# BaratiLab/MeshDQN

Hardware: AMD Instinct MI355X
Metric: env steps/sec (ys930 ~2k-tri) (higher is better)
Workload: dtype f64; 1 GPU; ys930 (876 vertices / 1570 triangles), 128 envs per GPU, S3 env step (remesh+smooth+interp+forces+state+1 IPCS step+Q-fwd); mesh=ys930, envs_per_gpu=128, parallelism=dp1 (independent envs sharded, no data-path collective)

## Files before the change

meshdqn_amd/csrc/mdq_ipcs_entry.hip:

```cpp
namespace mdq {

#ifdef MDQ_AT_TRACE
extern "C" MDQ_API int mdq_at_trace_host(long long* out, int reset) {
  if (hipMemcpyFromSymbol(out, HIP_SYMBOL(mdq_at_trace_buf), sizeof(long long) * 16) != hipSuccess) return -1;
  if (reset) { long long z[16] = {0}; if (hipMemcpyToSymbol(HIP_SYMBOL(mdq_at_trace_buf), z, sizeof z) != hipSuccess) return -1; }
  return 0;
}
extern "C" MDQ_API int mdq_pt_trace_host(long long* out, int reset) {
  if (hipMemcpyFromSymbol(out, HIP_SYMBOL(mdq_pt_trace_buf), sizeof(long long) * 16) != hipSuccess) return -1;
  if (reset) { long long z[16] = {0}; if (hipMemcpyToSymbol(HIP_SYMBOL(mdq_pt_trace_buf), z, sizeof z) != hipSuccess) return -1; }
  return 0;
}
extern "C" MDQ_API int mdq_ct_trace_host(long long* out, int reset) {
  if (hipMemcpyFromSymbol(out, HIP_SYMBOL(mdq_ct_trace_buf), sizeof(long long) * 16) != hipSuccess) return -1;
  if (reset) { long long z[16] = {0}; if (hipMemcpyToSymbol(HIP_SYMBOL(mdq_ct_trace_buf), z, sizeof z) != hipSuccess) return -1; }
  return 0;
}
#endif

static thread_local std::string g_err;

static int fail(const char* what, hipError_t e) {
  g_err = std::string(what) + ": " + hipGetErrorString(e);
  return -1;
// ... 66 lines not shown
  if (int rc = ensure_tables()) return rc;
  const size_t stage_bytes = 52 * (size_t)d->NT + 9 * (size_t)d->N2 + 9 * (size_t)d->NV + 64;
  hipError_t e;
  const size_t list_bytes = 2 * ((size_t)d->N2 + 1 + 6 * (size_t)d->NT + (size_t)d->NV + 1 + 3 * (size_t)d->NT) + 2;
  if (stage_bytes + list_bytes <= 156 * 1024 && 6 * (size_t)d->NT <= 65535) {
    const size_t bytes = stage_bytes + list_bytes;
    e = hipFuncSetAttribute(reinterpret_cast<const void*>(&setup_matfree_kernel<true, true>),
                            hipFuncAttributeMaxDynamicSharedMemorySize, (int)bytes);
    if (e != hipSuccess) return fail("setup_matfree_kernel attribute", e);
    hipLaunchKernelGGL((setup_matfree_kernel<true, true>), dim3(d->B), dim3(SWG), bytes, (hipStream_t)stream, *d);
  } else if (stage_bytes <= 156 * 1024) {
    e = hipFuncSetAttribute(reinterpret_cast<const void*>(&setup_matfree_kernel<true>), hipFuncAttributeMaxDynamicSharedMemorySize,
                            (int)stage_bytes);
    if (e != hipSuccess) return fail("setup_matfree_kernel attribute", e);
    hipLaunchKernelGGL(setup_matfree_kernel<true>, dim3(d->B), dim3(SWG), stage_bytes, (hipStream_t)stream, *d);
  } else if (const size_t idx_bytes = 12 * (size_t)d->NT + (size_t)d->N2 + 9 * (size_t)d->NV + 64;
             idx_bytes <= 156 * 1024 && d->N2 <= 65535 && std::getenv("MDQ_SETUP_UNSTAGED") == nullptr) {
    e = hipFuncSetAttribute(reinterpret_cast<const void*>(&setup_matfree_kernel<true, false, false>),
                            hipFuncAttributeMaxDynamicSharedMemorySize, (int)idx_bytes);
    if (e != hipSuccess) return fail("setup_matfree_kernel attribute", e);
    hipLaunchKernelGGL((setup_matfree_kernel<true, false, false>), dim3(d->B), dim3(SWG), idx_bytes, (hipStream_t)stream, *d);
  } else {
    hipLaunchKernelGGL(setup_matfree_kernel<false>, dim3(d->B), dim3(SWG), 0, (hipStream_t)stream, *d);
  }
  e = hipGetLastError();
  if (e != hipSuccess) return fail("setup_matfree_kernel launch", e);
  return 0;
}

static int ipcs_evolve_impl(const mdq_ipcs_desc* d, int32_t nsteps, double* drag, double* lift, int32_t* iters,
                            const double* inflow_scale, void* stream, double* kernel_ms, int fresh = 0,
                            const mdq_inflow_profile* prof = nullptr);

static int evolve_profile_checked(const char* entry, int fresh, const mdq_ipcs_desc* d, int32_t nsteps, double* drag, double* lift,
                                  int32_t* iters, const mdq_inflow_profile* prof, void* stream) {
  if (prof) {
    const auto bad = [entry](const char* what) { return fail_msg(std::string(entry) + what); };
    if (prof->NIN <= 0 || prof->NIR <= 0) return bad(": NIN and NIR must be positive");
    if (!prof->n_inlet || !prof->inlet_dofs || !prof->n_rows || !prof->rows || !prof->values)
      return bad(": incomplete inflow profile (n_inlet, inlet_dofs, n_rows, rows, values)");
    if (d && (!d->cell_dofs || !d->g2_ptr || !d->g2_src || !d->bcu_flag || !d->bcu_gx || !d->geom || !d->lift1 || !d->lift3))
      return bad(": incomplete descriptor (cell_dofs, g2_ptr, g2_src, bcu_flag, bcu_gx, geom, lift1, lift3)");
  }
  return ipcs_evolve_impl(d, nsteps, drag, lift, iters, nullptr, stream, nullptr, fresh, prof);
}

int mdq_ipcs_evolve_profile(const mdq_ipcs_desc* d, int32_t nsteps, double* drag, double* lift, int32_t* iters,
                            const mdq_inflow_profile* prof, void* stream) {
  return evolve_profile_checked("mdq_ipcs_evolve_profile", 0, d, nsteps, drag, lift, iters, prof, stream);
}

int mdq_ipcs_evolve_fresh_profile(const mdq_ipcs_desc* d, int32_t nsteps, double* drag, double* lift, int32_t* iters,
                                  const mdq_inflow_profile* prof, void* stream) {
  return evolve_profile_checked("mdq_ipcs_evolve_fresh_profile", 1, d, nsteps, drag, lift, iters, prof, stream);
}

int mdq_ipcs_build_inlet_map(const mdq_ipcs_desc* d, int32_t NIN, int32_t NIR, const int32_t* n_ref, const double* inlet_y,
                             int32_t* n_inlet, int32_t* inlet_dofs, int32_t* n_rows, int32_t* rows, int32_t* map_status,
                             void* stream) {
  if (!d || d->B <= 0 || d->NV <= 0 || d->NT <= 0 || d->NE <= 0 || d->N2 != d->NV + d->NE)
    return fail_msg("mdq_ipcs_build_inlet_map: bad batch sizes");
  if (!d->nv || !d->nt || !d->ne || !d->coords || !d->cell_dofs || !d->cell_outflow || !d->bcu_flag || !d->bcu_gx)
    return fail_msg("mdq_ipcs_build_inlet_map: incomplete descriptor (nv, nt, ne, coords, cell_dofs, cell_outflow, bcu_flag, bcu_gx)");
  if (d->N2 > MAP_BITS)
    return fail_msg("mdq_ipcs_build_inlet_map: N2 > " + std::to_string(MAP_BITS) + " (the inlet map serves the meshes of operator mode 3)");
  if (NIN <= 0 || NIN > MAP_NIN || NIR <= 0)
    return fail_msg("mdq_ipcs_build_inlet_map: NIN must be in 1 .. " + std::to_string(MAP_NIN) + " and NIR positive");
  if (!n_ref || !inlet_y || !n_inlet || !inlet_dofs || !n_rows || !rows || !map_status)
    return fail_msg("mdq_ipcs_build_inlet_map: null table (n_ref, inlet_y, n_inlet, inlet_dofs, n_rows, rows, map_status)");
  hipLaunchKernelGGL(inlet_map_kernel, dim3(d->B), dim3(MWG), 0, (hipStream_t)stream, *d, NIN, NIR, n_ref, inlet_y, n_inlet,
                     inlet_dofs, n_rows, rows, map_status);
  hipError_t e = hipGetLastError();
  if (e != hipSuccess) return fail("inlet_map_kernel launch", e);
  return 0;
}

int mdq_ipcs_evolve(const mdq_ipcs_desc* d, int32_t nsteps, double* drag, double* lift, int32_t* iters,
                    void* stream) {
  return ipcs_evolve_impl(d, nsteps, drag, lift, iters, nullptr, stream, nullptr);
}

int mdq_ipcs_evolve_inflow(const mdq_ipcs_desc* d, int32_t nsteps, double* drag, double* lift, int32_t* iters,
                           const double* inflow_scale, void* stream) {
  return ipcs_evolve_impl(d, nsteps, drag, lift, iters, inflow_scale, stream, nullptr);
}

int mdq_ipcs_evolve_fresh(const mdq_ipcs_desc* d, int32_t nsteps, double* drag, double* lift, int32_t* iters,
                          const double* inflow_scale, void* stream) {
  return ipcs_evolve_impl(d, nsteps, drag, lift, iters, inflow_scale, stream, nullptr, 1);
}

int mdq_ipcs_evolve_timed(const mdq_ipcs_desc* d, int32_t nsteps, double* drag, double* lift, int32_t* iters,
                          void* stream, double* kernel_ms) {
  if (!kernel_ms) return fail_msg("kernel_ms is required");
  if (d && d->mode != 3 && d->mode != -1) return fail_msg("per-kernel timing exists for the three-kernel mode 3 only");
  return ipcs_evolve_impl(d, nsteps, drag, lift, iters, nullptr, stream, kernel_ms);
}

static int ipcs_evolve_impl(const mdq_ipcs_desc* d, int32_t nsteps, double* drag, double* lift, int32_t* iters,
                            const double* inflow_scale, void* stream, double* kernel_ms, int fresh,
                            const mdq_inflow_profile* prof) {
  if (int rc = check_desc(d)) return rc;
  if (nsteps <= 0) return fail_msg("nsteps must be positive");
  if (!drag || !lift) return fail_msg("drag/lift output pointers are required");
  if (int rc = ensure_tables()) return rc;
  const LdsPlan P = lds_plan(d->N2, d->NV, d->NSE1);
  const size_t LDS_MAX = 160 * 1024, red_bytes = 64 * sizeof(double);
  const bool pg = red_bytes + P.prs_vec_bytes > LDS_MAX;
  const bool k1_lds = !pg && !d->pd_enabled && red_bytes + P.prs_vec_bytes + P.prs_mat_bytes <= LDS_MAX;
  int mode = d->mode;
  const size_t tile_bytes = tile_lds_bytes(*d);
  if (mode == 6) return fail_msg("unknown operator mode 6");
  if (mode < 0 || mode > 7) {
    mode = 0;
    if (red_bytes + P.vel1_bytes <= LDS_MAX) mode = 1;
    if (red_bytes + P.vel2_bytes <= LDS_MAX && d->N2 <= MF_ROWS * WG) mode = 2;
    if (d->mode != -2 && red_bytes + P.vel3_bytes <= LDS_MAX && d->N2 <= MF_ROWS * WG) mode = 3;
    if (mode == 0 && d->cell_outflow && ((d->mf_scat && d->mf_tptr) || (d->g2_ptr && d->g2_src)) && std::getenv("MDQ_NO_MODE5") == nullptr) mode = 5;
    if (mode == 0) {
      const int ncu = team_cus((hipStream_t)stream);
      if (!pg && 2 * TEAM * d->B <= ncu) mode = 4;
    }
    if (mode == 5 && !pg && std::getenv("MDQ_NO_TEAM_TILES") == nullptr) {
      if (TEAM * d->B <= team_cus((hipStream_t)stream)) mode = 7;
    }
  }
  if (kernel_ms && mode != 3) return fail_msg("per-kernel timing exists for the three-kernel mode 3 only");
  if (prof && mode != 2 && mode != 3)
    return fail_msg("mdq_ipcs_evolve_profile: operator mode " + std::to_string(mode) + " runs the steps of a call inside one kernel; "
                    "an inflow profile is served by the per-step path (operator modes 2 and 3, or mdq_ipcs_setup_matfree + "
                    "mdq_ipcs_evolve one step at a time)");
  if (fresh && mode != 3) {
    hipLaunchKernelGGL(reset_history_kernel, dim3((d->B + 63) / 64), dim3(64), 0, (hipStream_t)stream, *d, iters);
    if (hipError_t e_ = hipGetLastError(); e_ != hipSuccess) return fail("reset_history_kernel launch", e_);
  }
  if (mode == 3 && (red_bytes + P.vel3_bytes > LDS_MAX || d->N2 > MF_ROWS * WG))
    return fail_msg("mode 3 needs N2 <= 3584 and three velocity vectors in LDS");
  if (mode == 2 && (red_bytes + P.vel2_bytes > LDS_MAX || d->N2 > MF_ROWS * WG))
    return fail_msg("matrix-free tile mode needs N2 <= 3584 and the x stage + element tile in LDS");
  if (mode == 1 && red_bytes + P.vel1_bytes > LDS_MAX) return fail_msg("LDS gather vectors do not fit");
  if ((mode == 5 || mode == 7) && (!d->cell_outflow || !((d->mf_scat && d->mf_tptr) || (d->g2_ptr && d->g2_src))))
    return fail_msg("modes 5 / 7 need cell_outflow and the tile maps (mf_scat, mf_tptr) or the dof <- slot lists (g2_ptr, g2_src)");
  if (pg && mode != 0 && mode != 5)
    return fail_msg("mesh too large for the LDS-resident pressure vectors of this operator mode (use mode -1, 0 or 5)");
  size_t u = pg ? tl_extra_bytes(d->NV) + sizeof(double) * NAG * NAG : P.prs_vec_bytes + (k1_lds ? P.prs_mat_bytes : 0);
  const size_t vel = mode == 3 ? P.vel3_bytes : (mode == 2 ? P.vel2_bytes : (mode == 1 ? P.vel1_bytes : ((mode == 5 || mode == 7) ? tile_bytes : 0)));
  if (vel > u) u = vel;
  const size_t lds = red_bytes + u;
  hipError_t e;
  hipStream_t st = (hipStream_t)stream;
  if (mode == 3) {
    const size_t lds_v = red_bytes + P.vel3_bytes;
    const size_t lds_p = red_bytes + P.prs_vec_bytes + (k1_lds ? P.prs_mat_bytes : 0);
    const size_t lds_c = red_bytes + 2 * sizeof(double2) * (size_t)P.N2p + sizeof(double) * (size_t)P.NVp;
    static const hipError_t attr_err = [] {
      hipError_t e_ = hipFuncSetAttribute(reinterpret_cast<const void*>(&at_velocity_kernel<WG, MF_ROWS, AT_PAIR>),
                                          hipFuncAttributeMaxDynamicSharedMemorySize, 160 * 1024);
      if (e_ == hipSuccess)
        e_ = hipFuncSetAttribute(reinterpret_cast<const void*>(&at_velocity_kernel<768, 5, 1>),
                                 hipFuncAttributeMaxDynamicSharedMemorySize, 160 * 1024);
      if (e_ == hipSuccess)
        e_ = hipFuncSetAttribute(reinterpret_cast<const void*>(&at_pressure_kernel<true>),
                                 hipFuncAttributeMaxDynamicSharedMemorySize, 160 * 1024);
      if (e_ == hipSuccess)
        e_ = hipFuncSetAttribute(reinterpret_cast<const void*>(&at_pressure_kernel<false>),
                                 hipFuncAttributeMaxDynamicSharedMemorySize, 160 * 1024);
      if (e_ == hipSuccess)
        e_ = hipFuncSetAttribute(reinterpret_cast<const void*>(&at_pressure_kernel<false, 1024>),
                                 hipFuncAttributeMaxDynamicSharedMemorySize, 160 * 1024);
      if (e_ == hipSuccess)
        e_ = hipFuncSetAttribute(reinterpret_cast<const void*>(&at_correction_kernel),
                                 hipFuncAttributeMaxDynamicSharedMemorySize, 160 * 1024);
      return e_;
    }();
    if (attr_err != hipSuccess) return fail("hipFuncSetAttribute(mode 3 kernels)", attr_err);
    static const int vel_wg = [] {
      const char* s_ = std::getenv("MDQ_AT_WG");
      const int w_ = s_ ? std::atoi(s_) : 768;
      return w_ == 512 ? 512 : 768;
    }();
    hipEvent_t ev[4] = {nullptr, nullptr, nullptr, nullptr};
    if (kernel_ms) {
      for (int i = 0; i < 4; ++i)
        if ((e = hipEventCreate(&ev[i])) != hipSuccess) return fail("hipEventCreate", e);
      kernel_ms[0] = kernel_ms[1] = kernel_ms[2] = 0.0;
    }
    for (int step = 0; step < nsteps; ++step) {
      if (prof)
        if ((e = launch_inflow_lift(d, prof, nsteps, step, st)) != hipSuccess) return fail("inflow_lift_kernel launch", e);
      if (kernel_ms) hipEventRecord(ev[0], st);
      if (vel_wg == 768)
        hipLaunchKernelGGL((at_velocity_kernel<768, 5, 1>), dim3(d->B), dim3(768), lds_v, st, *d, iters, inflow_scale, nsteps, step, fresh);
      else
        hipLaunchKernelGGL((at_velocity_kernel<WG, MF_ROWS, AT_PAIR>), dim3(d->B), dim3(WG), lds_v, st, *d, iters, inflow_scale, nsteps, step, fresh);
      if (kernel_ms) hipEventRecord(ev[1], st);
      if (d->pd_enabled)
        hipLaunchKernelGGL((at_pressure_kernel<false, 1024>), dim3(d->B), dim3(1024), lds_p, st, *d, iters, fresh && step == 0);
      else if (k1_lds)
        hipLaunchKernelGGL(at_pressure_kernel<true>, dim3(d->B), dim3(WG), lds_p, st, *d, iters, fresh && step == 0);
      else
        hipLaunchKernelGGL(at_pressure_kernel<false>, dim3(d->B), dim3(WG), lds_p, st, *d, iters, fresh && step == 0);
      if (kernel_ms) hipEventRecord(ev[2], st);
      hipLaunchKernelGGL(at_correction_kernel, dim3(d->B), dim3(WG), lds_c, st, *d, nsteps, step, drag, lift, iters, inflow_scale, fresh);
      if (kernel_ms) {
        hipEventRecord(ev[3], st);
        if ((e = hipEventSynchronize(ev[3])) != hipSuccess) return fail("hipEventSynchronize", e);
        for (int i = 0; i < 3; ++i) {
          float ms = 0.f;
          hipEventElapsedTime(&ms, ev[i], ev[i + 1]);
          kernel_ms[i] += ms;
        }
      }
    }
    if (kernel_ms)
      for (int i = 0; i < 4; ++i) hipEventDestroy(ev[i]);
    e = hipGetLastError();
  } else {
    const EvolveArgs a{d, lds, nsteps, drag, lift, iters, inflow_scale, st, prof};
    if (mode == 2)
      e = part_launch_mf(k1_lds, a);
    else if (mode == 4 || mode == 5 || mode == 7)
      e = part_launch_tiles(mode, k1_lds, pg, a);
    else
      e = part_launch_assembled(mode, k1_lds, pg, a);
  }
  if (e != hipSuccess) return fail("evolve_kernel launch", e);
  return 0;
}

int mdq_probe_forces(const mdq_ipcs_desc* d, int32_t nfields, const double* u, const double* p, double* drag,
                     double* lift, void* stream) {
  if (!d || d->B <= 0 || d->N2 != d->NV + d->NE || !d->coords || !d->cell_dofs || !d->af_facets)
    return fail_msg("mdq_probe_forces: incomplete mesh descriptor");
  if (nfields <= 0 || !u || !p || !drag || !lift) return fail_msg("bad probe arguments");
  if (int rc = ensure_tables()) return rc;
  hipLaunchKernelGGL(probe_kernel, dim3(d->B), dim3(WG), 0, (hipStream_t)stream, *d, nfields, u, p, drag, lift);
  hipError_t e = hipGetLastError();
  if (e != hipSuccess) return fail("probe_kernel launch", e);
  return 0;
}

}
```

meshdqn_amd/csrc/mdq_ipcs_mode3.hip:

```cpp
#ifndef MDQ_CORR_MX0_INTERLEAVE
#define MDQ_CORR_MX0_INTERLEAVE false
#endif
#ifndef MDQ_PCG_REGM
#define MDQ_PCG_REGM 1
#endif
namespace mdq {

__device__ __forceinline__ double f2d(float f) {
  asm volatile("" : "+v"(f));
  return (double)f;
}


constexpr int AT_PAIR = 2;

template <int TPAIR = AT_PAIR>
struct AtMetaT {
  int w[TPAIR][6];
  Geo g[TPAIR];
};
using AtMeta = AtMetaT<AT_PAIR>;

template <int TW = WG, int TPAIR = AT_PAIR>
__device__ __forceinline__ void at_prefetch(const EnvView& v, AtMetaT<TPAIR>& m, int round) {
#pragma unroll
  for (int j = 0; j < TPAIR; ++j) {
    const int e = threadIdx.x + (round * TPAIR + j) * TW;
    if (e < v.nt) {
#pragma unroll
      for (int i = 0; i < 6; ++i) m.w[j][i] = v.mf_scat[i * v.NT + e];
      m.g[j] = load_geo(v, e);
    }
  }
}

template <bool INTERLEAVE, int TW = WG, int TPAIR = AT_PAIR, class ElemOp>
__device__ __forceinline__ void atomic_accumulate(const EnvView& v, double* Yd, AtMetaT<TPAIR>& m, ElemOp op) {
  const int nrounds = (v.nt + TPAIR * TW - 1) / (TPAIR * TW);
  for (int round = 0; round < nrounds; ++round) {
    if (INTERLEAVE) {
      double2 ye[TPAIR][6];
      int dof[TPAIR][6];
#pragma unroll
      for (int j = 0; j < TPAIR; ++j) {
        const int e = threadIdx.x + (round * TPAIR + j) * TW;
        if (e < v.nt) {
          ElemIdx E;
#pragma unroll
          for (int i = 0; i < 6; ++i) E.dof[i] = dof[j][i] = m.w[j][i] & 0xFFF;
          op(e, m.g[j], E, ((m.w[j][0] >> 28) & 3) - 1, ye[j]);
        }
      }
#pragma unroll
      for (int j = 0; j < TPAIR; ++j) {
        const int e = threadIdx.x + (round * TPAIR + j) * TW;
        if (e < v.nt) {
#pragma unroll
          for (int i = 0; i < 6; ++i) {
            unsafeAtomicAdd(Yd + 2 * dof[j][i], ye[j][i].x);
            unsafeAtomicAdd(Yd + 2 * dof[j][i] + 1, ye[j][i].y);
          }
        }
      }
    } else {
#pragma unroll 1
      for (int j = 0; j < TPAIR; ++j) {
        const int e = threadIdx.x + (round * TPAIR + j) * TW;
        if (e < v.nt) {
          ElemIdx E;
          double2 ye[6];
          const int* wj = (TPAIR == 1 || j == 0) ? m.w[0] : m.w[TPAIR - 1];
          const Geo gj = (TPAIR == 1 || j == 0) ? m.g[0] : m.g[TPAIR - 1];
#pragma unroll
          for (int i = 0; i < 6; ++i) E.dof[i] = wj[i] & 0xFFF;
          op(e, gj, E, ((wj[0] >> 28) & 3) - 1, ye);
#pragma unroll
          for (int i = 0; i < 6; ++i) {
            unsafeAtomicAdd(Yd + 2 * E.dof[i], ye[i].x);
            unsafeAtomicAdd(Yd + 2 * E.dof[i] + 1, ye[i].y);
          }
        }
      }
    }
    at_prefetch<TW, TPAIR>(v, m, round + 1 < nrounds ? round + 1 : 0);
  }
}

constexpr int BO_OWN = 2;
struct BoOwn {
  int t[BO_OWN];
};
template <int TW = WG>
__device__ __forceinline__ BoOwn outflow_rows_owned(const EnvView& v) {
  BoOwn o;
#pragma unroll
  for (int q = 0; q < BO_OWN; ++q) o.t[q] = -1;
  for (int t = 0; t < v.nbo; ++t) {
    if ((v.bo_rows[t] % TW) == (int)threadIdx.x) {
      if (o.t[0] < 0) o.t[0] = t;
      else o.t[1] = t;
    }
  }
  return o;
}

__device__ __forceinline__ void outflow_rows_add(const EnvView& v, const BoOwn& own, double coef, const double2* x,
                                                 double2* Y) {
#pragma unroll
  for (int q = 0; q < BO_OWN; ++q) {
    const int t = own.t[q];
    if (t >= 0) {
      const int row = v.bo_rows[t];
      double sx = 0.0, sy = 0.0;
      for (int k = v.bo_ptr[t]; k < v.bo_ptr[t + 1]; ++k) {
        const double4 bv = reinterpret_cast<const double4*>(v.bo_val)[k];
        const double2 xc = x[v.bo_col[k]];
        sx += bv.x * xc.x + bv.y * xc.y;
        sy += bv.z * xc.x + bv.w * xc.y;
      }
      const double2 y = Y[row];
      Y[row] = make_double2(y.x + coef * sx, y.y + coef * sy);
    }
  }
}


struct BoEnt {
  int rc;
  int nbe;
};
__device__ __forceinline__ int outflow_entry_rc(const EnvView& v, int t) {
  const int slot = v.bo_src[t];
  const int e = slot / 36, ij = slot - e * 36, i = ij / 6, j = ij - i * 6;
  return ((v.mf_scat[i * v.NT + e] & 0xFFF) << 12) | (v.mf_scat[j * v.NT + e] & 0xFFF);
}
__device__ __forceinline__ BoEnt outflow_entries_owned(const EnvView& v) {
  BoEnt o;
  o.nbe = v.nbo > 0 ? v.bo_ptr[v.nbo] : 0;
  o.rc = (int)threadIdx.x < o.nbe ? outflow_entry_rc(v, threadIdx.x) : -1;
  return o;
}
__device__ __forceinline__ void outflow_entry_apply(const EnvView& v, int t, int rc, double coef, const double2* x,
                                                    double* Yd) {
  const double4 bv = reinterpret_cast<const double4*>(v.bo_val)[t];
  const double2 xc = x[rc & 0xFFF];
  const int row = rc >> 12;
  unsafeAtomicAdd(Yd + 2 * row, coef * (bv.x * xc.x + bv.y * xc.y));
  unsafeAtomicAdd(Yd + 2 * row + 1, coef * (bv.z * xc.x + bv.w * xc.y));
}
template <int TW>
__device__ __forceinline__ void outflow_entries_add(const EnvView& v, const BoEnt& o, double coef, const double2* x,
                                                    double* Yd) {
  if (o.rc >= 0) outflow_entry_apply(v, threadIdx.x, o.rc, coef, x, Yd);
  for (int t = threadIdx.x + TW; t < o.nbe; t += TW) outflow_entry_apply(v, t, outflow_entry_rc(v, t), coef, x, Yd);
}


template <int TW, int TROWS, int TPAIR>
__global__ __launch_bounds__(TW) void at_velocity_kernel(mdq_ipcs_desc d, int32_t* iters, const double* inflow_scale, int nsteps,
                                                         int step, int fresh) {
  extern __shared__ __align__(16) double smem[];
  const int b = blockIdx.x, tid = threadIdx.x;
  const EnvView v = env_view(d, b);
  const double ai = inflow_factor(inflow_scale, b, nsteps, step);
  const int n2 = v.n2, nv = v.nv;
  const LdsPlan P = lds_plan(d.N2, d.NV, d.NSE1);
  const double a = uniform_double(v.rho / v.dt), mu = v.mu;
  (void)a; (void)mu; (void)nv; (void)n2;
  double* red = smem;
  double* U = smem + 64;
  double* w = v.work;
  double2* xs = reinterpret_cast<double2*>(w + 12 * (int64_t)d.NT);
  double* pnew = reinterpret_cast<double*>(xs + 6 * (int64_t)d.N2);
  int rsel = 0;
  (void)rsel; (void)pnew; (void)red;
  double2* Pl = reinterpret_cast<double2*>(U);
  double2* Rl = Pl + P.N2p;
  double2* Yl = Rl + P.N2p;
  double* Yd = reinterpret_cast<double*>(Yl);
  AtMetaT<TPAIR> tm;
  at_prefetch<TW, TPAIR>(v, tm, 0);
  const BoEnt bo_ent = outflow_entries_owned(v);
  int it_u = 0;
  double2* hist = xs + d.N2;
  double2* hist2 = xs + 2 * (int64_t)d.N2;
  double2* hist3 = xs + 4 * (int64_t)d.N2;
  double2* hist4 = xs + 5 * (int64_t)d.N2;
  double* histc = reinterpret_cast<double*>(xs + 3 * (int64_t)d.N2);
  const int nhist = (fresh && step == 0) ? 0 : (int)histc[0];
#ifdef MDQ_AT_TRACE
  long long tq_ = __builtin_amdgcn_s_memtime();
#endif
  __syncthreads();
  AT_STAMP(0)
  {
    int rc[TROWS];
    float2 idg[TROWS];
    unsigned flm = 0;
#pragma unroll
    for (int k = 0; k < TROWS; ++k) rc[k] = min(tid + k * TW, n2 - 1);
    {
      double2 un_[TROWS], dg_[TROWS];
      unsigned char fl_[TROWS];
#pragma unroll
      for (int k = 0; k < TROWS; ++k) {
        un_[k] = v.u_n[rc[k]];
        dg_[k] = v.idiag1[rc[k]];
        fl_[k] = v.bcu_flag[rc[k]];
      }
      double* Pn = reinterpret_cast<double*>(Rl);
      for (int i = tid; i < nv; i += TW) Pn[i] = v.p_n[i];
#pragma unroll
      for (int k = 0; k < TROWS; ++k) {
        const int row = tid + k * TW;
        idg[k] = (row < n2 && !fl_[k]) ? make_float2((float)dg_[k].x, (float)dg_[k].y) : make_float2(0.f, 0.f);
        flm |= fl_[k] ? 1u << k : 0u;
        if (row < n2) {
          Pl[row] = un_[k];
          Yl[row] = make_double2(0.0, 0.0);
        }
      }
    }
    __syncthreads();
    outflow_entries_add<TW>(v, bo_ent, 0.5 * mu, Pl, Yd);
    {
      const double* Pn = reinterpret_cast<const double*>(Rl);
      atomic_accumulate<false, TW, TPAIR>(v, Yd, tm, [&](int e, const Geo& g, const ElemIdx& E, int ko, double2(&ye)[6]) {
        double2 ue[6];
#pragma unroll
        for (int i = 0; i < 6; ++i) ue[i] = Pl[E.dof[i]];
        double pe[3];
#pragma unroll
        for (int i = 0; i < 3; ++i) pe[i] = Pn[E.dof[i]];
// ... 197 lines not shown
          AT_STAMP(9)
          double a3[2] = {0.0, 0.0};
          double2 t[TROWS];
#pragma unroll
          for (int k = 0; k < TROWS; ++k) {
            const int row = tid + k * TW;
            t[k] = make_double2(0.0, 0.0);
            if (row < n2) {
              const double2 yv = Yl[row], sv = Rl[row];
              t[k] = make_double2(yv.x * f2d(idg[k].x), yv.y * f2d(idg[k].y));
              a3[0] += t[k].x * sv.x + t[k].y * sv.y;
              a3[1] += t[k].x * t[k].x + t[k].y * t[k].y;
            }
          }
          block_sum1<2, TW / 64>(a3, red, rsel);
          AT_STAMP(10)
          if (a3[1] == 0.0) break;
          omega = a3[0] / a3[1];
          double a4[2] = {0.0, 0.0};
#pragma unroll
          for (int k = 0; k < TROWS; ++k) {
            const int row = tid + k * TW;
            if (row < n2) {
              const double2 pi = Pl[row], sv = Rl[row];
              xs[row] = make_double2(xo[k].x + alpha * pi.x + omega * sv.x, xo[k].y + alpha * pi.y + omega * sv.y);
              const double2 rn = make_double2(sv.x - omega * t[k].x, sv.y - omega * t[k].y);
              Rl[row] = rn;
              a4[0] += rn.x * rn.x + rn.y * rn.y;
              a4[1] += f2d(rh[k].x) * rn.x + f2d(rh[k].y) * rn.y;
            }
          }
          block_sum1<2, TW / 64>(a4, red, rsel);
          AT_STAMP(11)
          rr = a4[0];
          if (!(rr > tol2)) break;
          rho_old = rho;
          rho = a4[1];
          if (rho == 0.0 || omega == 0.0) break;
        }
        it_u += it;
      }
    }
    __syncthreads();
    AT_STAMP(12)
  }
  if (tid == 0) {
    histc[0] = (double)(nhist < 5 ? nhist + 1 : 5);
    if (iters) iters[3 * b + 0] = ((fresh && step == 0) ? 0 : iters[3 * b + 0]) + it_u;
  }
}

template <bool K1_LDS, int NTH = WG>
__global__ __launch_bounds__(NTH) void at_pressure_kernel(mdq_ipcs_desc d, int32_t* iters, int fresh) {
  extern __shared__ __align__(16) double smem[];
  const int b = blockIdx.x, tid = threadIdx.x;
  if (fresh && tid == 0 && iters) iters[3 * b + 1] = 0;
  const EnvView v = env_view(d, b);
  const int n2 = v.n2, nv = v.nv;
  const LdsPlan P = lds_plan(d.N2, d.NV, d.NSE1);
  const double a = v.rho / v.dt, mu = v.mu;
  (void)a; (void)mu; (void)nv; (void)n2;
  double* red = smem;
  double* U = smem + 64;
  double* w = v.work;
  double2* xs = reinterpret_cast<double2*>(w + 12 * (int64_t)d.NT);
  double* pnew = reinterpret_cast<double*>(xs + 6 * (int64_t)d.N2);
  int rsel = 0;
  (void)rsel; (void)pnew; (void)red;
  double* px = U;
  double* pr = px + P.NVp;
  double* pp = pr + P.NVp;
  double* pq = pp + P.NVp;
  double* lK = pq + P.NVp;
  int32_t* lci = reinterpret_cast<int32_t*>(lK + d.NSE1);
  int32_t* lso = lci + d.NSE1 + (d.NSE1 & 1);
  double* escr1 = w;
  const int nsl1 = (nv + 63) >> 6;
  const int32_t* so1 = K1_LDS ? lso : v.sl1_off;
  const int32_t* ci1 = K1_LDS ? lci : v.sl1_col;
  const double* K1 = K1_LDS ? lK : v.K1s;
  int it_p = 0;
#ifdef MDQ_AT_TRACE
  const long long tq0_ = __builtin_amdgcn_s_memtime();
#endif
  {
    if (K1_LDS && !d.pd_enabled) {
      const int ne1 = v.sl1_off[nsl1];
      for (int kk = tid; kk < ne1; kk += NTH) {
        lK[kk] = v.K1s[kk];
        lci[kk] = v.sl1_col[kk];
      }
      for (int kk = tid; kk <= nsl1; kk += NTH) lso[kk] = v.sl1_off[kk];
    }
    (void)escr1;
    for (int i = tid; i < nv; i += NTH) pr[i] = 0.0;
    __syncthreads();
    rhs2_accumulate_lds<NTH>(v, d, xs, v.p_n, pr);
    constexpr int PRW = 2048 / NTH;
    double sd_[PRW], pn_[PRW];
    unsigned fl_ = 0;
#pragma unroll
    for (int k = 0; k < PRW; ++k) {
      const int i = min(tid + k * NTH, nv - 1);
      sd_[k] = v.sdiagK[i];
      pn_[k] = v.p_n[i];
      fl_ |= v.bcp_flag[i] ? 1u << k : 0u;
    }
    __syncthreads();
#pragma unroll
    for (int k = 0; k < PRW; ++k) {
      const int i = tid + k * NTH;
      if (i < nv) {
        pr[i] = ((fl_ >> k) & 1u) ? 0.0 : pr[i] / sd_[k];
        px[i] = pn_[k] * sd_[k];
      }
    }
    for (int i = tid + PRW * NTH; i < nv; i += NTH) {
      const double sd = v.sdiagK[i];
      pr[i] = v.bcp_flag[i] ? 0.0 : pr[i] / sd;
      px[i] = v.p_n[i] * sd;
    }
    if (d.pd_enabled && d.pd_hdr[4 * (int64_t)b + 2] > 0) {
      const PdView pd = pd_view(d, b);
#ifdef MDQ_AT_TRACE
      { const long long tn_ = __builtin_amdgcn_s_memtime(); if (tid == 0 && b == 0) mdq_pt_trace_buf[0] += tn_ - tq0_; }
#endif
      pressure_direct<NTH>(pd, nv, pr, px, pp, pq, lK);
    } else {
      int itc = -1;
      if constexpr (NTH <= 512) {
        if (d.pcg_degree < 0)
          itc = cg_pressure_2l<NTH>(nv, so1, ci1, K1, v.coords, d.rtol, d.maxit_p, px, pr, pp, P.NVp, red, rsel);
        else if (nv <= 2 * NTH && d.pcg_degree > 0)
          itc = cg_pressure_cheb<NTH>(nv, so1, ci1, K1, d.rtol, d.maxit_p, d.pcg_degree, px, pr, pp, red, rsel);
        if (itc < 0 && nv <= 2 * NTH && d.pcg_degree == 0 && MDQ_PCG_REGM)
          itc = cg_pressure_regm<NTH>(nv, so1, ci1, K1, d.rtol, d.maxit_p, px, pr, pp, red, rsel);
      }
      if (itc >= 0)
        it_p += itc;
      else if (nv <= 2 * NTH)
        it_p += cg_pressure_reg<NTH>(nv, so1, ci1, K1, d.rtol, d.maxit_p, px, pr, pp, red, rsel);
      else
        it_p += cg_pressure(nv, so1, ci1, K1, d.rtol, d.maxit_p, px, pr, pp, pq, red);
    }
    for (int i = tid; i < nv; i += NTH) pnew[i] = px[i] / v.sdiagK[i];
    __syncthreads();

  }
  if (tid == 0 && iters) iters[3 * b + 1] += it_p;
}

static __global__ __launch_bounds__(WG) void at_correction_kernel(mdq_ipcs_desc d, int nsteps, int step, double* drag,
                                                            double* lift, int32_t* iters, const double* inflow_scale,
                                                            int fresh) {
  extern __shared__ __align__(16) double smem[];
  const int b = blockIdx.x, tid = threadIdx.x;
  const EnvView v = env_view(d, b);
  const double ai = inflow_factor(inflow_scale, b, nsteps, step);
  const bool fresh0 = fresh && step == 0;
  const int n2 = v.n2, nv = v.nv;
  const LdsPlan P = lds_plan(d.N2, d.NV, d.NSE1);
  const double a = v.rho / v.dt, mu = v.mu;
  (void)a; (void)mu; (void)nv; (void)n2;
  double* red = smem;
  double* U = smem + 64;
  double* w = v.work;
  double2* xs = reinterpret_cast<double2*>(w + 12 * (int64_t)d.NT);
  double* pnew = reinterpret_cast<double*>(xs + 6 * (int64_t)d.N2);
  int rsel = 0;
  (void)rsel; (void)pnew; (void)red;
  double2* Pl = reinterpret_cast<double2*>(U);
  double2* Yl = Pl + P.N2p;
  double* Yd = reinterpret_cast<double*>(Yl);
  AtMeta tm;
  at_prefetch(v, tm, 0);
  int it_m = 0;
  double2* cring = reinterpret_cast<double2*>(w + work_hist_offset(d.NV, d.NT, d.NE));
  double* ccnt = reinterpret_cast<double*>(cring + 3 * (int64_t)d.N2);
  const int nc = fresh0 ? 0 : (int)ccnt[0], rp = fresh0 ? 0 : (int)ccnt[1];
#ifdef MDQ_AT_TRACE
  long long tq_ = __builtin_amdgcn_s_memtime();
#endif
  __syncthreads();
  CT_STAMP(0)
  {
    double2 x[MF_ROWS], r[MF_ROWS], p[MF_ROWS];
    double ism[MF_ROWS];
    double am[2] = {0.0, 0.0};
    int rc[MF_ROWS];
#pragma unroll
    for (int k = 0; k < MF_ROWS; ++k) rc[k] = min(tid + k * WG, n2 - 1);
    double* Dp = reinterpret_cast<double*>(Yl + P.N2p);
    auto load_delta = [&](double2(&dl)[MF_ROWS]) {
#pragma unroll
      for (int k = 0; k < MF_ROWS; ++k) dl[k] = make_double2(0.0, 0.0);
      if (nc >= 1) {
        const double2* c1 = cring + (int64_t)((rp + 2) % 3) * d.N2;
        const double2* c2 = cring + (int64_t)((rp + 1) % 3) * d.N2;
        const double2* c3 = cring + (int64_t)rp * d.N2;
#pragma unroll
        for (int k = 0; k < MF_ROWS; ++k) dl[k] = c1[rc[k]];
        if (nc >= 2) {
          const double w1 = nc >= 3 ? 3.0 : 2.0, w2 = nc >= 3 ? -3.0 : -1.0;
#pragma unroll
          for (int k = 0; k < MF_ROWS; ++k) {
            const double2 b2 = c2[rc[k]];
            dl[k] = make_double2(w1 * dl[k].x + w2 * b2.x, w1 * dl[k].y + w2 * b2.y);
          }
          if (nc >= 3) {
#pragma unroll
            for (int k = 0; k < MF_ROWS; ++k) {
              const double2 b3 = c3[rc[k]];
              dl[k] = make_double2(dl[k].x + b3.x, dl[k].y + b3.y);
            }
          }
        }
      }
    };
    const double bb_lag = fresh0 ? 0.0 : ccnt[2];
    const int cstep = fresh0 ? 0 : (int)ccnt[3];
    const bool fused = nc >= 3 && bb_lag > 0.0 && (cstep & 15) != 0;
    {
      double2 us[MF_ROWS];
      if (!fused) {
#pragma unroll
        for (int k = 0; k < MF_ROWS; ++k) us[k] = xs[rc[k]];
      } else {
        load_delta(us);
#pragma unroll
        for (int k = 0; k < MF_ROWS; ++k) us[k] = make_double2(-us[k].x, -us[k].y);
      }
      for (int i = tid; i < nv; i += WG) Dp[i] = pnew[i] - v.p_n[i];
#pragma unroll
      for (int k = 0; k < MF_ROWS; ++k) {
        const int row = tid + k * WG;
        if (row < n2) {
          Pl[row] = us[k];
          Yl[row] = make_double2(0.0, 0.0);
        }
      }
    }
    __syncthreads();
    atomic_accumulate<true>(v, Yd, tm, [&](int, const Geo& g, const ElemIdx& E, int, double2(&ye)[6]) {
      double2 ue[6];
#pragma unroll
      for (int i = 0; i < 6; ++i) ue[i] = Pl[E.dof[i]];
      double dp[3];
#pragma unroll
      for (int i = 0; i < 3; ++i) dp[i] = Dp[E.dof[i]];
      elem_rhs3(g, v.dt, ue, dp, ye);
    });
    double2 l3[MF_ROWS], dlt[MF_ROWS];
    unsigned flm = 0;
    if (!fused) load_delta(dlt);
#pragma unroll
    for (int k = 0; k < MF_ROWS; ++k) {
      l3[k] = fused ? xs[rc[k]] : scaled2(ai, v.lift3[rc[k]]);
      ism[k] = v.sdiagM[rc[k]];
      flm |= v.bcu_flag[rc[k]] ? 1u << k : 0u;
    }
    __syncthreads();
    CT_STAMP(1)
    double bb;
    if (fused) {
#pragma unroll
      for (int k = 0; k < MF_ROWS; ++k) {
        r[k] = Yl[rc[k]];
        const double2 md = Pl[rc[k]];
        dlt[k] = make_double2(-md.x, -md.y);
      }
#pragma unroll
      for (int k = 0; k < MF_ROWS; ++k) {
        const int row = tid + k * WG;
        const bool fl = (flm >> k) & 1u;
        ism[k] = (row < n2 && !fl) ? 1.0 / ism[k] : 0.0;
        r[k] = make_double2(r[k].x * ism[k], r[k].y * ism[k]);
        p[k] = r[k];
        am[1] += r[k].x * r[k].x + r[k].y * r[k].y;
        x[k] = fl ? l3[k] : make_double2((l3[k].x + dlt[k].x) / (ism[k] != 0.0 ? ism[k] : 1.0),
                                          (l3[k].y + dlt[k].y) / (ism[k] != 0.0 ? ism[k] : 1.0));
        if (row >= n2) x[k] = make_double2(0.0, 0.0);
      }
      double a1r[1] = {am[1]};
      block_sum<1>(a1r, red);
      am[1] = a1r[0];
      bb = bb_lag;
      CT_STAMP(2)
      CT_STAMP(3)
    } else {
      double2 f3[MF_ROWS];
#pragma unroll
      for (int k = 0; k < MF_ROWS; ++k) {
        f3[k] = Yl[rc[k]];
        x[k] = Pl[rc[k]];
      }
#pragma unroll
      for (int k = 0; k < MF_ROWS; ++k) {
        const int row = tid + k * WG;
        const bool fl = (flm >> k) & 1u;
        ism[k] = (row < n2 && !fl) ? 1.0 / ism[k] : 0.0;
        if (!fl) x[k] = make_double2(x[k].x + dlt[k].x, x[k].y + dlt[k].y);
        if (row < n2) {
          Yl[row] = make_double2(0.0, 0.0);
          Pl[row] = x[k];
          const double2 bi = fl ? x[k] : make_double2((f3[k].x - l3[k].x) * ism[k], (f3[k].y - l3[k].y) * ism[k]);
          am[0] += bi.x * bi.x + bi.y * bi.y;
        } else {
          f3[k] = make_double2(0.0, 0.0);
        }
      }
      __syncthreads();
      CT_STAMP(2)
      atomic_accumulate<MDQ_CORR_MX0_INTERLEAVE>(v, Yd, tm, [&](int, const Geo& g, const ElemIdx& E, int, double2(&ye)[6]) {
        double2 xe[6];
#pragma unroll
        for (int i = 0; i < 6; ++i) xe[i] = Pl[E.dof[i]];
        elem_mass(g, xe, ye);
      });
      __syncthreads();
      CT_STAMP(3)
#pragma unroll
      for (int k = 0; k < MF_ROWS; ++k) {
        const int row = tid + k * WG;
        r[k] = p[k] = x[k] = make_double2(0.0, 0.0);
        if (row < n2) {
          const double2 ax = Yl[row];
          x[k] = Pl[row];
          r[k] = make_double2((f3[k].x - ax.x) * ism[k], (f3[k].y - ax.y) * ism[k]);
          p[k] = r[k];
          am[1] += r[k].x * r[k].x + r[k].y * r[k].y;
          if (ism[k] != 0.0) x[k] = make_double2(x[k].x / ism[k], x[k].y / ism[k]);
        }
      }
      block_sum<2>(am, red);
      bb = am[0];
      if (tid == 0) ccnt[2] = bb;
    }
    CT_STAMP(4)
    {
      const double tol2 = d.rtol * d.rtol * bb;
      double rr = am[1];
      if (rr > tol2 && bb != 0.0) {
        int it = 0;
        while (it < d.maxit_m) {
          ++it;
#pragma unroll
          for (int k = 0; k < MF_ROWS; ++k) {
            const int row = tid + k * WG;
            if (row < n2) {
              Pl[row] = make_double2(p[k].x * ism[k], p[k].y * ism[k]);
              Yl[row] = make_double2(0.0, 0.0);
            }
          }
          __syncthreads();
          CT_STAMP(5)
          atomic_accumulate<true>(v, Yd, tm, [&](int, const Geo& g, const ElemIdx& E, int, double2(&ye)[6]) {
            double2 xe[6];
#pragma unroll
            for (int i = 0; i < 6; ++i) xe[i] = Pl[E.dof[i]];
            elem_mass(g, xe, ye);
          });
          __syncthreads();
          CT_STAMP(6)
          double a1[1] = {0.0};
          double2 q[MF_ROWS];
#pragma unroll
          for (int k = 0; k < MF_ROWS; ++k) {
            const int row = tid + k * WG;
            q[k] = make_double2(0.0, 0.0);
            if (row < n2) {
              const double2 yv = Yl[row];
              q[k] = make_double2(yv.x * ism[k], yv.y * ism[k]);
              a1[0] += p[k].x * q[k].x + p[k].y * q[k].y;
            }
          }
          block_sum1<1>(a1, red, rsel);
          CT_STAMP(7)
          if (!(a1[0] > 0.0)) break;
          const double alpha = rr / a1[0];
          double a2[1] = {0.0};
#pragma unroll
          for (int k = 0; k < MF_ROWS; ++k) {
            x[k] = make_double2(x[k].x + alpha * p[k].x, x[k].y + alpha * p[k].y);
            r[k] = make_double2(r[k].x - alpha * q[k].x, r[k].y - alpha * q[k].y);
            a2[0] += r[k].x * r[k].x + r[k].y * r[k].y;
          }
          block_sum1<1>(a2, red, rsel);
          CT_STAMP(8)
          const double rr_new = a2[0];
          if (!(rr_new > tol2)) break;
          const double beta = rr_new / rr;
          rr = rr_new;
#pragma unroll
          for (int k = 0; k < MF_ROWS; ++k)
            p[k] = make_double2(r[k].x + beta * p[k].x, r[k].y + beta * p[k].y);
        }
        it_m += it;
      }
    }

    {
      double2 us[MF_ROWS];
#pragma unroll
      for (int k = 0; k < MF_ROWS; ++k) us[k] = xs[rc[k]];
      double2* cnew = cring + (int64_t)rp * d.N2;
#pragma unroll
      for (int k = 0; k < MF_ROWS; ++k) {
        const int row = tid + k * WG;
        if (row < n2) {
          const double2 un = (ism[k] != 0.0) ? make_double2(x[k].x * ism[k], x[k].y * ism[k]) : x[k];
          v.u_n[row] = un;
          cnew[row] = (ism[k] != 0.0) ? make_double2(un.x - us[k].x, un.y - us[k].y) : make_double2(0.0, 0.0);
        }
      }
    }
    if (tid == 0) {
      ccnt[0] = (double)(nc < 3 ? nc + 1 : 3);
      ccnt[1] = (double)((rp + 1) % 3);
      ccnt[3] = (double)((cstep + 1) & 1023);
      if (fresh0) {
        double* hcnt = reinterpret_cast<double*>(cring + 5 * (int64_t)d.N2);
        hcnt[0] = hcnt[1] = 0.0;
      }
    }
    for (int i = tid; i < nv; i += WG) v.p_n[i] = pnew[i];
    __syncthreads();
    CT_STAMP(9)
    double dr, li;
    forces(v, v.mu, v.u_n, v.p_n, red, dr, li);
    CT_STAMP(10)
    if (tid == 0) {
      drag[(int64_t)b * nsteps + step] = dr;
      lift[(int64_t)b * nsteps + step] = li;
    }
  }
  if (tid == 0 && iters) iters[3 * b + 2] = (fresh0 ? 0 : iters[3 * b + 2]) + it_m;
}

}
```

Before: 187,700 env steps/s.

## Replace edge-DOF LDS atomics with owner/secondary slot writes in correction kernel

In the correction kernel, each mesh edge (a P2 midpoint DOF) is shared by at most two triangles. The kernel now computes an owner triangle per edge once, using atomicMin in LDS. Edge contributions are then written with plain stores: the owner writes into the main accumulator and the second triangle writes into an extra per-edge slot array in LDS. Row reads add the two values, so the double-precision LDS atomics for three of the six DOFs per element are replaced by plain stores in the RHS and mass-matrix (CG) scatters. The cost is extra LDS of NE double2, a setup pass per launch, an extra read per edge row, and more register use. An env-var switch can disable it or exclude one env for debugging.

```diff
diff --git a/meshdqn_amd/csrc/mdq_ipcs_entry.hip b/meshdqn_amd/csrc/mdq_ipcs_entry.hip
--- a/meshdqn_amd/csrc/mdq_ipcs_entry.hip
+++ b/meshdqn_amd/csrc/mdq_ipcs_entry.hip
@@ -242,7 +242,14 @@
   if (mode == 3) {
     const size_t lds_v = red_bytes + P.vel3_bytes;
     const size_t lds_p = red_bytes + P.prs_vec_bytes + (k1_lds ? P.prs_mat_bytes : 0);
-    const size_t lds_c = red_bytes + 2 * sizeof(double2) * (size_t)P.N2p + sizeof(double) * (size_t)P.NVp;
+    size_t lds_c = red_bytes + 2 * sizeof(double2) * (size_t)P.N2p + sizeof(double) * (size_t)P.NVp;
+    static const int corr_edge = [] {
+      const char* s_ = std::getenv("MDQ_CORR_EDGE_PARENT");
+      return s_ ? std::atoi(s_) : 0;
+    }();
+    const int corr_slots = (corr_edge <= 0 && lds_c + sizeof(double2) * (size_t)d->NE <= LDS_MAX) ? 1 : 0;
+    if (corr_slots) lds_c += sizeof(double2) * (size_t)d->NE;
+    const int corr_parent_env = corr_edge < 0 ? -corr_edge - 1 : -1;
     static const hipError_t attr_err = [] {
       hipError_t e_ = hipFuncSetAttribute(reinterpret_cast<const void*>(&at_velocity_kernel<WG, MF_ROWS, AT_PAIR>),
                                           hipFuncAttributeMaxDynamicSharedMemorySize, 160 * 1024);
@@ -291,7 +298,7 @@
       else
         hipLaunchKernelGGL(at_pressure_kernel<false>, dim3(d->B), dim3(WG), lds_p, st, *d, iters, fresh && step == 0);
       if (kernel_ms) hipEventRecord(ev[2], st);
-      hipLaunchKernelGGL(at_correction_kernel, dim3(d->B), dim3(WG), lds_c, st, *d, nsteps, step, drag, lift, iters, inflow_scale, fresh);
+      hipLaunchKernelGGL(at_correction_kernel, dim3(d->B), dim3(WG), lds_c, st, *d, nsteps, step, drag, lift, iters, inflow_scale, fresh, corr_slots, corr_parent_env);
       if (kernel_ms) {
         hipEventRecord(ev[3], st);
         if ((e = hipEventSynchronize(ev[3])) != hipSuccess) return fail("hipEventSynchronize", e);
diff --git a/meshdqn_amd/csrc/mdq_ipcs_mode3.hip b/meshdqn_amd/csrc/mdq_ipcs_mode3.hip
--- a/meshdqn_amd/csrc/mdq_ipcs_mode3.hip
+++ b/meshdqn_amd/csrc/mdq_ipcs_mode3.hip
@@ -34,8 +34,49 @@
   }
 }
 
-template <bool INTERLEAVE, int TW = WG, int TPAIR = AT_PAIR, class ElemOp>
-__device__ __forceinline__ void atomic_accumulate(const EnvView& v, double* Yd, AtMetaT<TPAIR>& m, ElemOp op) {
+constexpr int ES_MAX_TRI = 10;
+struct EdgeSlots {
+  double2* E2;
+  int nv;
+  unsigned sec;
+  bool on;
+};
+
+__device__ __forceinline__ double2 edge_row_sum(const EdgeSlots& es, const double2* Yl, int row) {
+  double2 y = Yl[row];
+  if (es.on && row >= es.nv) {
+    const double2 s = es.E2[row - es.nv];
+    y = make_double2(y.x + s.x, y.y + s.y);
+  }
+  return y;
+}
+
+template <bool ESLOT>
+__device__ __forceinline__ void at_scatter(double* Yd, const int (&dof)[6], int t, const double2 (&ye)[6], const EdgeSlots* es) {
+  if (ESLOT && es->on) {
+#pragma unroll
+    for (int i = 0; i < 3; ++i) {
+      unsafeAtomicAdd(Yd + 2 * dof[i], ye[i].x);
+      unsafeAtomicAdd(Yd + 2 * dof[i] + 1, ye[i].y);
+    }
+    const unsigned sec = es->sec >> (3 * t);
+#pragma unroll
+    for (int i = 3; i < 6; ++i) {
+      double2* dst = ((sec >> (i - 3)) & 1u) ? es->E2 + (dof[i] - es->nv) : reinterpret_cast<double2*>(Yd) + dof[i];
+      *dst = ye[i];
+    }
+  } else {
+#pragma unroll
+    for (int i = 0; i < 6; ++i) {
+      unsafeAtomicAdd(Yd + 2 * dof[i], ye[i].x);
+      unsafeAtomicAdd(Yd + 2 * dof[i] + 1, ye[i].y);
+    }
+  }
+}
+
+template <bool INTERLEAVE, int TW = WG, int TPAIR = AT_PAIR, bool ESLOT = false, class ElemOp>
+__device__ __forceinline__ void atomic_accumulate(const EnvView& v, double* Yd, AtMetaT<TPAIR>& m, ElemOp op,
+                                                  const EdgeSlots* es = nullptr) {
   const int nrounds = (v.nt + TPAIR * TW - 1) / (TPAIR * TW);
   for (int round = 0; round < nrounds; ++round) {
     if (INTERLEAVE) {
@@ -54,13 +95,7 @@
 #pragma unroll
       for (int j = 0; j < TPAIR; ++j) {
         const int e = threadIdx.x + (round * TPAIR + j) * TW;
-        if (e < v.nt) {
-#pragma unroll
-          for (int i = 0; i < 6; ++i) {
-            unsafeAtomicAdd(Yd + 2 * dof[j][i], ye[j][i].x);
-            unsafeAtomicAdd(Yd + 2 * dof[j][i] + 1, ye[j][i].y);
-          }
-        }
+        if (e < v.nt) at_scatter<ESLOT>(Yd, dof[j], round * TPAIR + j, ye[j], es);
       }
     } else {
 #pragma unroll 1
@@ -74,11 +109,7 @@
 #pragma unroll
           for (int i = 0; i < 6; ++i) E.dof[i] = wj[i] & 0xFFF;
           op(e, gj, E, ((wj[0] >> 28) & 3) - 1, ye);
-#pragma unroll
-          for (int i = 0; i < 6; ++i) {
-            unsafeAtomicAdd(Yd + 2 * E.dof[i], ye[i].x);
-            unsafeAtomicAdd(Yd + 2 * E.dof[i] + 1, ye[i].y);
-          }
+          at_scatter<ESLOT>(Yd, E.dof, round * TPAIR + j, ye, es);
         }
       }
     }
@@ -582,7 +613,7 @@
 
 static __global__ __launch_bounds__(WG) void at_correction_kernel(mdq_ipcs_desc d, int nsteps, int step, double* drag,
                                                             double* lift, int32_t* iters, const double* inflow_scale,
-                                                            int fresh) {
+                                                            int fresh, int slots, int parent_env) {
   extern __shared__ __align__(16) double smem[];
   const int b = blockIdx.x, tid = threadIdx.x;
   const EnvView v = env_view(d, b);
@@ -605,6 +636,54 @@
   AtMeta tm;
   at_prefetch(v, tm, 0);
   int it_m = 0;
+  EdgeSlots es;
+  es.E2 = Yl + P.N2p + P.NVp / 2;
+  es.nv = nv;
+  es.sec = 0u;
+  es.on = slots && b != parent_env && v.nt > 0 && v.nt <= ES_MAX_TRI * WG;
+  if (es.on) {
+    int* eown = reinterpret_cast<int*>(es.E2);
+    int* bad = reinterpret_cast<int*>(red);
+    int ed[ES_MAX_TRI][3];
+#pragma unroll
+    for (int t = 0; t < ES_MAX_TRI; ++t) {
+      const int e = tid + t * WG, ec = min(e, v.nt - 1);
+#pragma unroll
+      for (int i = 0; i < 3; ++i) {
+        const int w_ = v.mf_scat[(3 + i) * v.NT + ec];
+        ed[t][i] = e < v.nt ? (w_ & 0xFFF) - nv : -1;
+      }
+    }
+    for (int i = tid; i < v.ne; i += WG) eown[i] = 0x7FFFFFFF;
+    if (tid == 0) *bad = 0;
+    __syncthreads();
+#pragma unroll
+    for (int t = 0; t < ES_MAX_TRI; ++t) {
+      const int e = tid + t * WG;
+      if (e < v.nt) {
+#pragma unroll
+        for (int i = 0; i < 3; ++i) {
+          if ((unsigned)ed[t][i] < (unsigned)v.ne) atomicMin(&eown[ed[t][i]], e);
+          else *bad = 1;
+        }
+      }
+    }
+    __syncthreads();
+    es.on = *bad == 0;
+    if (es.on) {
+#pragma unroll
+      for (int t = 0; t < ES_MAX_TRI; ++t) {
+        const int e = tid + t * WG;
+        if (e < v.nt) {
+#pragma unroll
+          for (int i = 0; i < 3; ++i)
+            if (eown[ed[t][i]] != e) es.sec |= 1u << (3 * t + i);
+        }
+      }
+    }
+    __syncthreads();
+    for (int i = tid; i < v.ne; i += WG) es.E2[i] = make_double2(0.0, 0.0);
+  }
   double2* cring = reinterpret_cast<double2*>(w + work_hist_offset(d.NV, d.NT, d.NE));
   double* ccnt = reinterpret_cast<double*>(cring + 3 * (int64_t)d.N2);
   const int nc = fresh0 ? 0 : (int)ccnt[0], rp = fresh0 ? 0 : (int)ccnt[1];
@@ -671,7 +750,7 @@
       }
     }
     __syncthreads();
-    atomic_accumulate<true>(v, Yd, tm, [&](int, const Geo& g, const ElemIdx& E, int, double2(&ye)[6]) {
+    atomic_accumulate<true, WG, AT_PAIR, true>(v, Yd, tm, [&](int, const Geo& g, const ElemIdx& E, int, double2(&ye)[6]) {
       double2 ue[6];
 #pragma unroll
       for (int i = 0; i < 6; ++i) ue[i] = Pl[E.dof[i]];
@@ -679,7 +758,7 @@
 #pragma unroll
       for (int i = 0; i < 3; ++i) dp[i] = Dp[E.dof[i]];
       elem_rhs3(g, v.dt, ue, dp, ye);
-    });
+    }, &es);
     double2 l3[MF_ROWS], dlt[MF_ROWS];
     unsigned flm = 0;
     if (!fused) load_delta(dlt);
@@ -695,7 +774,7 @@
     if (fused) {
 #pragma unroll
       for (int k = 0; k < MF_ROWS; ++k) {
-        r[k] = Yl[rc[k]];
+        r[k] = edge_row_sum(es, Yl, rc[k]);
         const double2 md = Pl[rc[k]];
         dlt[k] = make_double2(-md.x, -md.y);
       }
@@ -721,7 +800,7 @@
       double2 f3[MF_ROWS];
 #pragma unroll
       for (int k = 0; k < MF_ROWS; ++k) {
-        f3[k] = Yl[rc[k]];
+        f3[k] = edge_row_sum(es, Yl, rc[k]);
         x[k] = Pl[rc[k]];
       }
 #pragma unroll
@@ -741,12 +820,12 @@
       }
       __syncthreads();
       CT_STAMP(2)
-      atomic_accumulate<MDQ_CORR_MX0_INTERLEAVE>(v, Yd, tm, [&](int, const Geo& g, const ElemIdx& E, int, double2(&ye)[6]) {
+      atomic_accumulate<MDQ_CORR_MX0_INTERLEAVE, WG, AT_PAIR, true>(v, Yd, tm, [&](int, const Geo& g, const ElemIdx& E, int, double2(&ye)[6]) {
         double2 xe[6];
 #pragma unroll
         for (int i = 0; i < 6; ++i) xe[i] = Pl[E.dof[i]];
         elem_mass(g, xe, ye);
-      });
+      }, &es);
       __syncthreads();
       CT_STAMP(3)
 #pragma unroll
@@ -754,7 +833,7 @@
         const int row = tid + k * WG;
         r[k] = p[k] = x[k] = make_double2(0.0, 0.0);
         if (row < n2) {
-          const double2 ax = Yl[row];
+          const double2 ax = edge_row_sum(es, Yl, row);
           x[k] = Pl[row];
           r[k] = make_double2((f3[k].x - ax.x) * ism[k], (f3[k].y - ax.y) * ism[k]);
           p[k] = r[k];
@@ -784,12 +863,12 @@
           }
           __syncthreads();
           CT_STAMP(5)
-          atomic_accumulate<true>(v, Yd, tm, [&](int, const Geo& g, const ElemIdx& E, int, double2(&ye)[6]) {
+          atomic_accumulate<true, WG, AT_PAIR, true>(v, Yd, tm, [&](int, const Geo& g, const ElemIdx& E, int, double2(&ye)[6]) {
             double2 xe[6];
 #pragma unroll
             for (int i = 0; i < 6; ++i) xe[i] = Pl[E.dof[i]];
             elem_mass(g, xe, ye);
-          });
+          }, &es);
           __syncthreads();
           CT_STAMP(6)
           double a1[1] = {0.0};
@@ -799,7 +878,7 @@
             const int row = tid + k * WG;
             q[k] = make_double2(0.0, 0.0);
             if (row < n2) {
-              const double2 yv = Yl[row];
+              const double2 yv = edge_row_sum(es, Yl, row);
               q[k] = make_double2(yv.x * ism[k], yv.y * ism[k]);
               a1[0] += p[k].x * q[k].x + p[k].y * q[k].y;
             }
```

Measured after the change: 187,900 env steps/s, median of 5. Within noise of the previous version (+0.1%).
